# bowang-lab/BioReason

Measured on NVIDIA H100. Metric: GRPO tokens/sec (rollout+update), higher is better.
Workload: dtype bf16

## Files before the change

### bioreason_b200/csrc/br_common.cuh

```cuda
#pragma once
#include <cuda_runtime.h>
#include <cuda_bf16.h>
#include <cuda.h>
#include <stdint.h>
#include <stdio.h>
#include <string.h>
#include <stdlib.h>

#define BR_OK 0
#define BR_ERR_INVALID (-1)
#define BR_ERR_CUDA (-2)
#define BR_ERR_UNSUPPORTED (-3)

void br_set_error(const char* fmt, ...);

#define BR_CHECK_ARG(cond, ...)                     \
    do {                                            \
        if (!(cond)) {                              \
            br_set_error(__VA_ARGS__);              \
            return BR_ERR_INVALID;                  \
        }                                           \
    } while (0)

#define BR_CHECK_CUDA(expr)                                                              \
    do {                                                                                 \
        cudaError_t _e = (expr);                                                         \
        if (_e != cudaSuccess) {                                                         \
            br_set_error("%s failed: %s (%s:%d)", #expr, cudaGetErrorString(_e), __FILE__, __LINE__); \
            return BR_ERR_CUDA;                                                          \
        }                                                                                \
    } while (0)

#define BR_CHECK_LAUNCH() BR_CHECK_CUDA(cudaGetLastError())

static inline int br_num_sms() {
    static int n = 0;
    if (!n) {
        int dev = 0;
        cudaGetDevice(&dev);
        cudaDeviceGetAttribute(&n, cudaDevAttrMultiProcessorCount, dev);
        if (n <= 0) n = 132;
    }
    return n;
}

typedef __nv_bfloat16 bf16;
typedef __nv_bfloat162 bf162;

#ifdef __CUDACC__
namespace br {

__device__ __forceinline__ uint32_t smem_u32(const void* p) { return (uint32_t)__cvta_generic_to_shared(p); }
__device__ __forceinline__ int lane_id() { return threadIdx.x & 31; }

__device__ __forceinline__ void mbar_init(uint64_t* bar, uint32_t count) {
    asm volatile("mbarrier.init.shared::cta.b64 [%0], %1;" ::"r"(smem_u32(bar)), "r"(count));
}
__device__ __forceinline__ void mbar_fence_init() { asm volatile("fence.mbarrier_init.release.cluster;" ::: "memory"); }
__device__ __forceinline__ void mbar_expect_tx(uint64_t* bar, uint32_t bytes) {
    asm volatile("mbarrier.arrive.expect_tx.shared::cta.b64 _, [%0], %1;" ::"r"(smem_u32(bar)), "r"(bytes) : "memory");
}
__device__ __forceinline__ void mbar_arrive(uint64_t* bar) {
    asm volatile("mbarrier.arrive.shared::cta.b64 _, [%0];" ::"r"(smem_u32(bar)) : "memory");
}
__device__ __forceinline__ void mbar_wait(uint64_t* bar, uint32_t parity) {
    asm volatile(
        "{\n"
        ".reg .pred p;\n"
        "WAIT_%=:\n"
        "mbarrier.try_wait.parity.shared::cta.b64 p, [%0], %1;\n"
        "@p bra DONE_%=;\n"
        "bra WAIT_%=;\n"
        "DONE_%=:\n"
        "}\n" ::"r"(smem_u32(bar)),
        "r"(parity)
        : "memory");
}

__device__ __forceinline__ void tma_prefetch_desc(const void* tmap) {
    asm volatile("prefetch.tensormap [%0];" ::"l"(tmap) : "memory");
}
__device__ __forceinline__ void tma_load_2d(void* smem_dst, const void* tmap, uint64_t* bar, int c0, int c1) {
    asm volatile(
        "cp.async.bulk.tensor.2d.shared::cluster.global.mbarrier::complete_tx::bytes [%0], [%1, {%3, %4}], [%2];" ::"r"(
            smem_u32(smem_dst)),
        "l"(tmap), "r"(smem_u32(bar)), "r"(c0), "r"(c1)
        : "memory");
}

__device__ __forceinline__ void tma_load_2d_hint(void* smem_dst, const void* tmap, uint64_t* bar, int c0, int c1, uint64_t policy) {
    asm volatile(
        "cp.async.bulk.tensor.2d.shared::cluster.global.mbarrier::complete_tx::bytes.L2::cache_hint [%0], [%1, {%3, %4}], [%2], %5;" ::"r"(
            smem_u32(smem_dst)),
        "l"(tmap), "r"(smem_u32(bar)), "r"(c0), "r"(c1), "l"(policy)
        : "memory");
}
__device__ __forceinline__ void bulk_load_hint(void* smem_dst, const void* src, uint32_t bytes, uint64_t* bar, uint64_t policy) {
    asm volatile(
        "cp.async.bulk.shared::cluster.global.mbarrier::complete_tx::bytes.L2::cache_hint [%0], [%1], %2, [%3], %4;" ::"r"(smem_u32(smem_dst)),
        "l"(src), "r"(bytes), "r"(smem_u32(bar)), "l"(policy)
        : "memory");
}
__device__ __forceinline__ uint64_t make_policy_evict_first() {
    uint64_t p; asm volatile("createpolicy.fractional.L2::evict_first.b64 %0, 1.0;" : "=l"(p)); return p;
}

__device__ __forceinline__ void fence_proxy_async_smem() { asm volatile("fence.proxy.async.shared::cta;" ::: "memory"); }

__device__ __forceinline__ void launch_dependents() { asm volatile("griddepcontrol.launch_dependents;" ::: "memory"); }
__device__ __forceinline__ void grid_dep_wait() { asm volatile("griddepcontrol.wait;" ::: "memory"); }

__device__ __forceinline__ float warp_sum(float v) {
#pragma unroll
    for (int o = 16; o > 0; o >>= 1) v += __shfl_xor_sync(0xffffffffu, v, o);
    return v;
}
__device__ __forceinline__ float warp_max(float v) {
#pragma unroll
    for (int o = 16; o > 0; o >>= 1) v = fmaxf(v, __shfl_xor_sync(0xffffffffu, v, o));
    return v;
}
__device__ __forceinline__ uint32_t pack_bf16(float lo, float hi) {
    bf162 t = __floats2bfloat162_rn(lo, hi);
    return *reinterpret_cast<uint32_t*>(&t);
}
__device__ __forceinline__ float2 unpack_bf16(uint32_t v) {
    bf162 t = *reinterpret_cast<bf162*>(&v);
    return __bfloat1622float2(t);
}

__device__ __forceinline__ uint4 philox4x32_10(uint4 c, uint32_t k0, uint32_t k1) {
#pragma unroll
    for (int i = 0; i < 10; ++i) {
        if (i) { k0 += 0x9E3779B9u; k1 += 0xBB67AE85u; }
        const uint32_t hi0 = __umulhi(0xD2511F53u, c.x), lo0 = 0xD2511F53u * c.x;
        const uint32_t hi1 = __umulhi(0xCD9E8D57u, c.z), lo1 = 0xCD9E8D57u * c.z;
        c = make_uint4(hi1 ^ c.y ^ k0, lo1, hi0 ^ c.w ^ k1, lo0);
    }
    return c;
}

}
#endif

#ifdef __CUDACC__
template <typename... KArgs, typename... Args>
static inline cudaError_t br_launch_pdl(void (*kern)(KArgs...), dim3 grid, dim3 block, size_t smem, cudaStream_t st, Args&&... args) {
    cudaLaunchConfig_t cfg = {};
    cfg.gridDim = grid; cfg.blockDim = block; cfg.dynamicSmemBytes = smem; cfg.stream = st;
    static const bool no_pdl = getenv("BR_NO_PDL") != nullptr;
    cudaLaunchAttribute attr[1];
    attr[0].id = cudaLaunchAttributeProgrammaticStreamSerialization;
    attr[0].val.programmaticStreamSerializationAllowed = 1;
    cfg.attrs = attr; cfg.numAttrs = no_pdl ? 0 : 1;
    return cudaLaunchKernelEx(&cfg, kern, static_cast<KArgs>(args)...);
}
#endif

int br_make_tmap_2d_bf16(CUtensorMap* out, const void* base, uint64_t rows, uint64_t cols, uint64_t ld_elems, uint32_t box_rows);
```

### bioreason_b200/csrc/gemm_tc5.cu

```cuda
#include "br_common.cuh"
#include "../../include/bioreason_b200.h"
#include "lora_dropout.cuh"
#include "wgmma.cuh"

namespace {

constexpr int BM = 128;
constexpr int BK = 64;
constexpr int NTHREADS = 288;

enum { MODE_STD = 0, MODE_LSE = 1, MODE_DLOGITS = 2 };

struct GemmParams {
    int M, N, K, K2;
    int ldd;
    void* D;
    const void* bias; int bias_f32;
    const bf16* residual; long long ldr;
    float alpha;
    int act;
    int out_f32;
    const int* row_map;
    bf16* aux; long long ld_aux;
    const int* target;
    float* pmax; float* psum; float* tgt_logit;
    const float* lse; const float* gscale;
    int n_tiles_m, n_tiles_n;
    int group_m;
    br::DropParams drop;
};

template <int BN>
struct SmemLayout {
    static constexpr int A_BYTES = BM * BK * 2;
    static constexpr int B_BYTES = BN * BK * 2;
    static constexpr int STAGE_BYTES = A_BYTES + B_BYTES;
    static constexpr int NSTAGE = BN == 128 ? 6 : 4;
    static constexpr int TILE_BYTES = NSTAGE * STAGE_BYTES;
    static constexpr int TOTAL = TILE_BYTES + 256 + 1024;
};

__device__ __forceinline__ void tile_coords(int tile, int ntm, int ntn, int GROUP_M, int& mb, int& nb) {
    int per_group = GROUP_M * ntn;
    int g = tile / per_group;
    int first_m = g * GROUP_M;
    int gsize = min(GROUP_M, ntm - first_m);
    int r = tile - g * per_group;
    mb = first_m + (r % gsize);
    nb = r / gsize;
}

__device__ __forceinline__ float rbf(float x) { return __bfloat162float(__float2bfloat16(x)); }

template <int BN>
__device__ __forceinline__ void masked_segment(float (&acc)[BN / 2], uint64_t adesc, uint64_t bdesc, int k0, int mb, int nb, int wg,
                                               const GemmParams& p) {
    const int lane = threadIdx.x & 31, q = lane & 3;
    const long long grow = p.drop.row0 + mb * BM + wg * 64 + ((threadIdx.x >> 5) & 3) * 16 + (lane >> 2);
    const int cg0 = (nb * BN) >> 3;
    br::wg_wait<0>();
    br::wg_fence_operand(acc);
    for (int kk = 0; kk < BK / 16;) {
        const int kc = k0 + 16 * kk;
        if (kc >= p.K2) break;
        const int jb = kc / p.drop.r;
        const int nk = min(p.drop.r - (kc - jb * p.drop.r), BK - 16 * kk) >> 4;
        float tmp[BN / 2];
#pragma unroll
        for (int i = 0; i < BN / 2; ++i) tmp[i] = 0.f;
        br::wg_fence();
        for (int t = 0; t < nk; ++t) br::wgmma_ss<BN>(tmp, adesc + 2 * (kk + t), bdesc + 2 * (kk + t), 1);
        br::wg_commit();
        br::wg_wait<0>();
        br::wg_fence_operand(tmp);
        const int j = p.drop.proj + jb;
#pragma unroll
        for (int set = 0; set < BN / 16; ++set) {
            uint32_t w[4];
            br::quad_words(br::drop_group(p.drop, grow + 8 * (q & 1), cg0 + 2 * set + (q >> 1), j), w);
#pragma unroll
            for (int g = 0; g < 4; ++g) {
                const int e = 4 * (2 * set + (g >> 1)) + 2 * (g & 1);
                acc[e] += br::keep_lo(w[g], p.drop.T) ? tmp[e] * p.drop.inv_keep : 0.f;
                acc[e + 1] += br::keep_hi(w[g], p.drop.T) ? tmp[e + 1] * p.drop.inv_keep : 0.f;
            }
        }
        kk += nk;
    }
}

template <int BN, int MODE, bool MASK>
__global__ void __launch_bounds__(NTHREADS, 1)
gemm_tc5_kernel(const __grid_constant__ CUtensorMap tmA, const __grid_constant__ CUtensorMap tmB,
                const __grid_constant__ CUtensorMap tmA2, const __grid_constant__ CUtensorMap tmB2,
                const GemmParams p) {
    static_assert(BN == 128 || BN == 256, "tile width");
    static_assert(!MASK || BN == 128, "the masked LoRA segment runs on 128-wide tiles");
    constexpr int NSUB = BN / 128;
    using L = SmemLayout<BN>;
    extern __shared__ uint8_t smem_raw[];
    uint8_t* smem = reinterpret_cast<uint8_t*>((reinterpret_cast<uintptr_t>(smem_raw) + 1023) & ~uintptr_t(1023));
    uint64_t* full_bar = reinterpret_cast<uint64_t*>(smem + L::TILE_BYTES);
    uint64_t* empty_bar = full_bar + L::NSTAGE;

    const int warp = threadIdx.x >> 5;
    const int lane = threadIdx.x & 31;
    const int num_tiles = p.n_tiles_m * ((p.n_tiles_n + NSUB - 1) / NSUB);
    const int kb1 = (p.K + BK - 1) / BK;
    const int kb2 = (p.K2 + BK - 1) / BK;
    const int num_kb = kb1 + kb2;

    if (threadIdx.x == 0) {
        br::tma_prefetch_desc(&tmA);
        br::tma_prefetch_desc(&tmB);
        if (kb2) { br::tma_prefetch_desc(&tmA2); br::tma_prefetch_desc(&tmB2); }
        for (int s = 0; s < L::NSTAGE; ++s) { br::mbar_init(&full_bar[s], 1); br::mbar_init(&empty_bar[s], 2); }
        br::mbar_fence_init();
    }
    __syncthreads();

    if (warp == 8) {
        if (lane == 0) {
            int s = 0; uint32_t ph = 0;
            for (int tile = blockIdx.x; tile < num_tiles; tile += gridDim.x) {
                int mb, nb; tile_coords(tile, p.n_tiles_m, (p.n_tiles_n + NSUB - 1) / NSUB, p.group_m, mb, nb);
                for (int kb = 0; kb < num_kb; ++kb) {
                    br::mbar_wait(&empty_bar[s], ph ^ 1);
                    uint8_t* sa = smem + s * L::STAGE_BYTES;
                    uint8_t* sb = sa + L::A_BYTES;
                    br::mbar_expect_tx(&full_bar[s], L::STAGE_BYTES);
                    if (kb < kb1) {
                        br::tma_load_2d(sa, &tmA, &full_bar[s], kb * BK, mb * BM);
                        br::tma_load_2d(sb, &tmB, &full_bar[s], kb * BK, nb * BN);
                    } else {
                        br::tma_load_2d(sa, &tmA2, &full_bar[s], (kb - kb1) * BK, mb * BM);
                        br::tma_load_2d(sb, &tmB2, &full_bar[s], (kb - kb1) * BK, nb * BN);
                    }
                    if (++s == L::NSTAGE) { s = 0; ph ^= 1; }
                }
            }
        }
        return;
    }
    const int wg = warp >> 2;
    const int wt = threadIdx.x & 127;
    int s = 0; uint32_t ph = 0;
    for (int tile = blockIdx.x; tile < num_tiles; tile += gridDim.x) {
        int mb, nb; tile_coords(tile, p.n_tiles_m, (p.n_tiles_n + NSUB - 1) / NSUB, p.group_m, mb, nb);
        float acc[BN / 2];
#pragma unroll
        for (int i = 0; i < BN / 2; ++i) acc[i] = 0.f;
        int prev = 0;
        for (int kb = 0; kb < num_kb; ++kb) {
            br::mbar_wait(&full_bar[s], ph);
            const uint32_t sa = br::smem_u32(smem + s * L::STAGE_BYTES);
            const uint64_t adesc = br::wg_desc_k(sa + wg * 64 * 128);
            const uint64_t bdesc = br::wg_desc_k(sa + L::A_BYTES);
            if constexpr (MASK) {
                if (kb >= kb1) {
                    masked_segment<BN>(acc, adesc, bdesc, (kb - kb1) * BK, mb, nb, wg, p);
                    if (wt == 0) br::mbar_arrive(&empty_bar[prev]);
                    prev = s;
                    if (++s == L::NSTAGE) { s = 0; ph ^= 1; }
                    continue;
                }
            }
            br::wg_fence();
#pragma unroll
            for (int k = 0; k < BK / 16; ++k) br::wgmma_ss<BN>(acc, adesc + 2 * k, bdesc + 2 * k, 1);
            br::wg_commit();
            if (kb > 0) {
                br::wg_wait<1>();
                if (wt == 0) br::mbar_arrive(&empty_bar[prev]);
            }
            prev = s;
            if (++s == L::NSTAGE) { s = 0; ph ^= 1; }
        }
        br::wg_wait<0>();
        br::wg_fence_operand(acc);
        if (wt == 0) br::mbar_arrive(&empty_bar[prev]);

        const int r0 = mb * BM + wg * 64 + (warp & 3) * 16 + (lane >> 2);
        const int n0 = nb * BN;
        const int cq = 2 * (lane & 3);
        if constexpr (MODE == MODE_STD) {
#pragma unroll
            for (int hh = 0; hh < 2; ++hh) {
                const int row = r0 + 8 * hh;
                if (row >= p.M) continue;
                const long long orow = p.row_map ? (long long)p.row_map[row] : (long long)row;
                if (orow < 0) continue;
                float v[BN / 4];
#pragma unroll
                for (int i = 0; i < BN / 8; ++i) {
                    v[2 * i] = acc[4 * i + 2 * hh] * p.alpha;
                    v[2 * i + 1] = acc[4 * i + 2 * hh + 1] * p.alpha;
                    const int col = n0 + 8 * i + cq;
                    if (p.bias && n0 + 8 * i < p.N) {
                        if (p.bias_f32) {
                            const float* b = reinterpret_cast<const float*>(p.bias) + col;
                            v[2 * i] += __ldg(b); v[2 * i + 1] += __ldg(b + 1);
                        } else {
                            const bf16* b = reinterpret_cast<const bf16*>(p.bias) + col;
                            v[2 * i] += __bfloat162float(b[0]); v[2 * i + 1] += __bfloat162float(b[1]);
                        }
                    }
                }
                if (p.act == 1) {
#pragma unroll
                    for (int j = 0; j < BN / 16; ++j) {
                        if (n0 + 16 * j >= p.N) break;
                        if (p.aux) {
                            bf16* a = p.aux + orow * p.ld_aux + n0 + 16 * j + cq;
                            *reinterpret_cast<uint32_t*>(a) = br::pack_bf16(v[4 * j], v[4 * j + 1]);
                            *reinterpret_cast<uint32_t*>(a + 8) = br::pack_bf16(v[4 * j + 2], v[4 * j + 3]);
                        }
                        float o[2];
#pragma unroll
                        for (int e = 0; e < 2; ++e) {
                            const float g = rbf(v[4 * j + e]), u = rbf(v[4 * j + 2 + e]);
                            o[e] = rbf(g / (1.f + __expf(-g))) * u;
                        }
                        bf16* d = reinterpret_cast<bf16*>(p.D) + orow * (long long)p.ldd + (n0 >> 1) + 8 * j + cq;
                        *reinterpret_cast<uint32_t*>(d) = br::pack_bf16(o[0], o[1]);
                    }
                    continue;
                }
#pragma unroll
                for (int i = 0; i < BN / 8; ++i) {
                    if (n0 + 8 * i >= p.N) break;
                    const int col = n0 + 8 * i + cq;
                    float x0 = v[2 * i], x1 = v[2 * i + 1];
                    if (p.residual) {
                        const float2 r = br::unpack_bf16(__ldg(reinterpret_cast<const unsigned int*>(p.residual + orow * p.ldr + col)));
                        x0 = rbf(x0) + r.x; x1 = rbf(x1) + r.y;
                    }
                    if (p.out_f32) *reinterpret_cast<float2*>(reinterpret_cast<float*>(p.D) + orow * (long long)p.ldd + col) = make_float2(x0, x1);
                    else *reinterpret_cast<uint32_t*>(reinterpret_cast<bf16*>(p.D) + orow * (long long)p.ldd + col) = br::pack_bf16(x0, x1);
                }
            }
        } else if constexpr (MODE == MODE_LSE) {
#pragma unroll
            for (int h = 0; h < NSUB; ++h) {
                const int nh = n0 + 128 * h;
                if (NSUB > 1 && nh >= p.N) break;
#pragma unroll
                for (int hh = 0; hh < 2; ++hh) {
                    const int row = r0 + 8 * hh;
                    const bool row_ok = row < p.M;
                    const int tgt = row_ok ? p.target[row] : -1;
                    float mx = -INFINITY;
#pragma unroll
                    for (int i = 0; i < 16; ++i)
                        if (nh + 8 * i < p.N) mx = fmaxf(mx, fmaxf(acc[64 * h + 4 * i + 2 * hh], acc[64 * h + 4 * i + 2 * hh + 1]) * p.alpha);
                    mx = fmaxf(mx, __shfl_xor_sync(0xffffffffu, mx, 1));
                    mx = fmaxf(mx, __shfl_xor_sync(0xffffffffu, mx, 2));
                    float sm = 0.f;
#pragma unroll
                    for (int i = 0; i < 16; ++i) {
                        if (nh + 8 * i >= p.N) continue;
                        const int col = nh + 8 * i + cq;
                        const float x0 = acc[64 * h + 4 * i + 2 * hh] * p.alpha, x1 = acc[64 * h + 4 * i + 2 * hh + 1] * p.alpha;
                        sm += __expf(x0 - mx) + __expf(x1 - mx);
                        if (col == tgt) p.tgt_logit[row] = x0;
                        if (col + 1 == tgt) p.tgt_logit[row] = x1;
                    }
                    sm += __shfl_xor_sync(0xffffffffu, sm, 1);
                    sm += __shfl_xor_sync(0xffffffffu, sm, 2);
                    if (row_ok && (lane & 3) == 0) {
                        p.pmax[(long long)row * p.n_tiles_n + nb * NSUB + h] = mx;
                        p.psum[(long long)row * p.n_tiles_n + nb * NSUB + h] = sm;
                    }
                }
            }
        } else {
#pragma unroll
            for (int hh = 0; hh < 2; ++hh) {
                const int row = r0 + 8 * hh;
                if (row >= p.M) continue;
                const int tgt = p.target[row];
                const float lse = p.lse[row], gs = p.gscale[row];
#pragma unroll
                for (int i = 0; i < BN / 8; ++i) {
                    if (n0 + 8 * i >= p.N) break;
                    const int col = n0 + 8 * i + cq;
                    const float d0 = gs * ((col == tgt ? 1.f : 0.f) - __expf(acc[4 * i + 2 * hh] * p.alpha - lse));
                    const float d1 = gs * ((col + 1 == tgt ? 1.f : 0.f) - __expf(acc[4 * i + 2 * hh + 1] * p.alpha - lse));
                    *reinterpret_cast<uint32_t*>(reinterpret_cast<bf16*>(p.D) + (long long)row * p.ldd + col) = br::pack_bf16(d0, d1);
                }
            }
        }
    }
}

__global__ void lse_combine_kernel(const float* __restrict__ pmax, const float* __restrict__ psum, const float* __restrict__ tgt_logit,
                                   const int* __restrict__ target, int M, int nt, float* __restrict__ lse, float* __restrict__ logp) {
    int row = blockIdx.x * (blockDim.x >> 5) + (threadIdx.x >> 5);
    if (row >= M) return;
    int lane = threadIdx.x & 31;
    float mx = -INFINITY;
    for (int t = lane; t < nt; t += 32) mx = fmaxf(mx, pmax[(long long)row * nt + t]);
    mx = br::warp_max(mx);
    float s = 0.f;
    for (int t = lane; t < nt; t += 32) s += psum[(long long)row * nt + t] * __expf(pmax[(long long)row * nt + t] - mx);
    s = br::warp_sum(s);
    if (lane == 0) {
        float l = logf(s) + mx;
        if (lse) lse[row] = l;
        if (logp) logp[row] = (target[row] >= 0) ? tgt_logit[row] - l : 0.f;
    }
}

typedef CUresult (*PFN_encodeTiled)(CUtensorMap*, CUtensorMapDataType, cuuint32_t, void*, const cuuint64_t*, const cuuint64_t*,
                                    const cuuint32_t*, const cuuint32_t*, CUtensorMapInterleave, CUtensorMapSwizzle,
                                    CUtensorMapL2promotion, CUtensorMapFloatOOBfill);
PFN_encodeTiled get_encode() {
    static PFN_encodeTiled fn = nullptr;
    if (!fn) {
        void* f = nullptr;
        cudaDriverEntryPointQueryResult q;
        if (cudaGetDriverEntryPoint("cuTensorMapEncodeTiled", &f, cudaEnableDefault, &q) == cudaSuccess && q == cudaDriverEntryPointSuccess)
            fn = reinterpret_cast<PFN_encodeTiled>(f);
    }
    return fn;
}

template <int BN, int MODE, bool MASK = false>
int launch(const CUtensorMap& a, const CUtensorMap& b, const CUtensorMap& a2, const CUtensorMap& b2, const GemmParams& p, cudaStream_t st) {
    auto kern = gemm_tc5_kernel<BN, MODE, MASK>;
    static bool attr_set = false;
    if (!attr_set) {
        BR_CHECK_CUDA(cudaFuncSetAttribute(kern, cudaFuncAttributeMaxDynamicSharedMemorySize, SmemLayout<BN>::TOTAL));
        attr_set = true;
    }
    int tiles = p.n_tiles_m * ((p.n_tiles_n + BN / 128 - 1) / (BN / 128));
    int grid = tiles < br_num_sms() ? tiles : br_num_sms();
    kern<<<grid, NTHREADS, SmemLayout<BN>::TOTAL, st>>>(a, b, a2, b2, p);
    BR_CHECK_LAUNCH();
    return BR_OK;
}

template <int BN>
int launch_mode(int mode, const CUtensorMap& a, const CUtensorMap& b, const CUtensorMap& a2, const CUtensorMap& b2, const GemmParams& p,
                cudaStream_t st) {
    if (mode == MODE_STD) return launch<BN, MODE_STD>(a, b, a2, b2, p, st);
    if (mode == MODE_LSE) return launch<BN, MODE_LSE>(a, b, a2, b2, p, st);
    return launch<BN, MODE_DLOGITS>(a, b, a2, b2, p, st);
}

int run_gemm(int mode, const void* A, int64_t lda, const void* B, int64_t ldb, int M, int N, int K, const void* A2, int64_t lda2,
             const void* B2, int64_t ldb2, int K2, GemmParams& p, cudaStream_t st, bool masked = false) {
    BR_CHECK_ARG(M > 0 && N > 0 && K > 0, "gemm: empty problem M=%d N=%d K=%d", M, N, K);
    BR_CHECK_ARG(N % 8 == 0 && K % 8 == 0 && lda % 8 == 0 && ldb % 8 == 0, "gemm: N, K, lda, ldb must be multiples of 8");
    BR_CHECK_ARG(((uintptr_t)A % 16 == 0) && ((uintptr_t)B % 16 == 0), "gemm: operands must be 16-byte aligned");
    p.M = M; p.N = N; p.K = K; p.K2 = (A2 && B2) ? K2 : 0;
    p.n_tiles_m = (M + BM - 1) / BM;
    p.n_tiles_n = (N + 127) / 128;
    const bool wide = !masked && N >= 256 && K >= 512 && (long long)p.n_tiles_m * ((N + 255) / 256) >= 2ll * br_num_sms();
    const int bn = wide ? 256 : 128;
    {
        const long long a_block = (long long)BM * (K + p.K2) * 2;
        long long g = (16ll << 20) / (a_block > 0 ? a_block : 1);
        if (g < 8) g = 8;
        if (g > p.n_tiles_m) g = p.n_tiles_m;
        p.group_m = (int)g;
    }
    CUtensorMap ta, tb, ta2, tb2;
    int rc;
    if ((rc = br_make_tmap_2d_bf16(&ta, A, M, K, lda, BM))) return rc;
    if ((rc = br_make_tmap_2d_bf16(&tb, B, N, K, ldb, bn))) return rc;
    if (p.K2) {
        BR_CHECK_ARG(K2 % 8 == 0 && lda2 % 8 == 0 && ldb2 % 8 == 0, "gemm: K2, lda2, ldb2 must be multiples of 8");
        if ((rc = br_make_tmap_2d_bf16(&ta2, A2, M, K2, lda2, BM))) return rc;
        if ((rc = br_make_tmap_2d_bf16(&tb2, B2, N, K2, ldb2, bn))) return rc;
    } else { ta2 = ta; tb2 = tb; }
    if (masked) return launch<128, MODE_STD, true>(ta, tb, ta2, tb2, p, st);
    return wide ? launch_mode<256>(mode, ta, tb, ta2, tb2, p, st) : launch_mode<128>(mode, ta, tb, ta2, tb2, p, st);
}

}

int br_make_tmap_2d_bf16(CUtensorMap* out, const void* base, uint64_t rows, uint64_t cols, uint64_t ld_elems, uint32_t box_rows) {
    PFN_encodeTiled enc = get_encode();
    if (!enc) { br_set_error("cuTensorMapEncodeTiled not available from the driver"); return BR_ERR_CUDA; }
    cuuint64_t gdim[2] = {cols, rows};
    cuuint64_t gstr[1] = {ld_elems * 2};
    cuuint32_t box[2] = {64, box_rows};
    cuuint32_t estr[2] = {1, 1};
    CUresult r = enc(out, CU_TENSOR_MAP_DATA_TYPE_BFLOAT16, 2, const_cast<void*>(base), gdim, gstr, box, estr, CU_TENSOR_MAP_INTERLEAVE_NONE,
                     CU_TENSOR_MAP_SWIZZLE_128B, CU_TENSOR_MAP_L2_PROMOTION_L2_256B, CU_TENSOR_MAP_FLOAT_OOB_FILL_NONE);
    if (r != CUDA_SUCCESS) {
        br_set_error("cuTensorMapEncodeTiled failed (%d) rows=%llu cols=%llu ld=%llu box_rows=%u base=%p", (int)r, (unsigned long long)rows,
                     (unsigned long long)cols, (unsigned long long)ld_elems, box_rows, base);
        return BR_ERR_CUDA;
    }
    return BR_OK;
}

extern "C" {

int br_gemm_bf16(const void* A, int64_t lda, const void* B, int64_t ldb, void* D, int64_t ldd, int M, int N, int K,
                 const br_gemm_epilogue* e, void* stream) {
    GemmParams p;
    memset(&p, 0, sizeof(p));
    p.D = D; p.ldd = (int)ldd; p.alpha = 1.f;
    const void *A2 = nullptr, *B2 = nullptr; int64_t lda2 = 0, ldb2 = 0; int K2 = 0;
    bool masked = false;
    if (e) {
        p.bias = e->bias; p.bias_f32 = e->bias_dtype == BR_F32;
        p.residual = reinterpret_cast<const bf16*>(e->residual); p.ldr = e->ldr;
        p.alpha = e->alpha; p.act = e->act; p.out_f32 = e->out_dtype == BR_F32;
        p.row_map = e->row_map; p.aux = reinterpret_cast<bf16*>(e->aux_out); p.ld_aux = e->ld_aux;
        A2 = e->A2; B2 = e->B2; lda2 = e->lda2; ldb2 = e->ldb2; K2 = e->K2;
        BR_CHECK_ARG(!(p.act == 1 && (p.out_f32 || p.residual)), "gemm: gated-SiLU epilogue writes bf16 without residual");
        BR_CHECK_ARG(!(p.act == 1 && N % 16 != 0), "gemm: gated-SiLU epilogue needs N %% 16 == 0");
        if (e->lora_dropout) {
            int rc;
            if ((rc = br::check_drop(e->lora_dropout, "gemm"))) return rc;
            const int r = e->lora_dropout->r;
            BR_CHECK_ARG(A2 && B2 && r % 16 == 0 && r > 0 && K2 % r == 0 && e->lora_dropout->proj + K2 / r <= 8,
                         "gemm: masked LoRA segment needs A2/B2 with K2 = n_proj * r, r %% 16 == 0 (K2=%d r=%d)", K2, r);
            BR_CHECK_ARG(!p.row_map, "gemm: masked LoRA segment indexes mask rows by input row; no row_map");
            p.drop = br::drop_params(*e->lora_dropout);
            masked = true;
        }
    }
    BR_CHECK_ARG(ldd % 8 == 0 && (uintptr_t)D % 16 == 0, "gemm: D must be 16-byte aligned with ldd %% 8 == 0");
    return run_gemm(MODE_STD, A, lda, B, ldb, M, N, K, A2, lda2, B2, ldb2, K2, p, (cudaStream_t)stream, masked);
}

int64_t br_lmhead_workspace_bytes(int M, int V) {
    int nt = (V + 127) / 128;
    return (int64_t)M * nt * 2 * sizeof(float) + (int64_t)M * sizeof(float);
}

int br_lmhead_logprob_fwd(const void* H, int64_t ldh, const void* W, int64_t ldw, const int32_t* target, int M, int V, int K, float scale,
                          float* logp, float* lse, void* workspace, void* stream) {
    GemmParams p;
    memset(&p, 0, sizeof(p));
    int nt_max = (V + 127) / 128;
    p.alpha = scale; p.target = target;
    p.pmax = reinterpret_cast<float*>(workspace);
    p.psum = p.pmax + (int64_t)M * nt_max;
    p.tgt_logit = p.psum + (int64_t)M * nt_max;
    cudaStream_t st = (cudaStream_t)stream;
    BR_CHECK_CUDA(cudaMemsetAsync(p.tgt_logit, 0, (size_t)M * sizeof(float), st));
    int rc = run_gemm(MODE_LSE, H, ldh, W, ldw, M, V, K, nullptr, 0, nullptr, 0, 0, p, st);
    if (rc) return rc;
    const int wpb = 8;
    lse_combine_kernel<<<(M + wpb - 1) / wpb, wpb * 32, 0, st>>>(p.pmax, p.psum, p.tgt_logit, target, M, p.n_tiles_n, lse, logp);
    BR_CHECK_LAUNCH();
    return BR_OK;
}

int br_lmhead_dlogits(const void* H, int64_t ldh, const void* W, int64_t ldw, const int32_t* target, const float* lse, const float* gscale,
                      int M, int V, int K, float scale, void* dlogits, int64_t ldd, void* stream) {
    GemmParams p;
    memset(&p, 0, sizeof(p));
    p.alpha = scale; p.target = target; p.lse = lse; p.gscale = gscale; p.D = dlogits; p.ldd = (int)ldd;
    BR_CHECK_ARG(ldd % 8 == 0, "lmhead_dlogits: ldd %% 8");
    return run_gemm(MODE_DLOGITS, H, ldh, W, ldw, M, V, K, nullptr, 0, nullptr, 0, 0, p, (cudaStream_t)stream);
}

}
```

Measured before the change: 1224.

## Add 2-CTA cluster ping-pong WGMMA GEMM with multicast B and vectorized epilogue

Adds a new persistent GEMM kernel for wide standard-mode GEMMs with K up to 4096. It pairs CTAs in a cluster of two that share the B tile through TMA multicast, and runs two consumer warpgroups in ping-pong on alternating tiles so one tile's epilogue overlaps the other's MMA. Register reallocation via setmaxnreg favours the consumer warpgroups. The epilogue is factored out and now uses quad-shuffle transposes to emit 16-byte stores instead of 4-byte ones. This adds cross-CTA barrier complexity and lowers occupancy to one CTA per SM.

```diff
diff --git a/bioreason_b200/csrc/br_common.cuh b/bioreason_b200/csrc/br_common.cuh
--- a/bioreason_b200/csrc/br_common.cuh
+++ b/bioreason_b200/csrc/br_common.cuh
@@ -77,6 +77,20 @@
         : "memory");
 }
 
+__device__ __forceinline__ uint32_t cluster_ctarank() {
+    uint32_t r; asm volatile("mov.u32 %0, %%cluster_ctarank;" : "=r"(r)); return r;
+}
+__device__ __forceinline__ void cluster_sync() { asm volatile("barrier.cluster.arrive;\nbarrier.cluster.wait;" ::: "memory"); }
+__device__ __forceinline__ void mbar_arrive_cluster(uint64_t* bar, uint32_t cta) {
+    asm volatile("{\n.reg .b32 ra;\nmapa.shared::cluster.u32 ra, %0, %1;\nmbarrier.arrive.shared::cluster.b64 _, [ra];\n}" ::"r"(
+                     smem_u32(bar)), "r"(cta)
+                 : "memory");
+}
+template <int R> __device__ __forceinline__ void setmaxnreg_inc() { asm volatile("setmaxnreg.inc.sync.aligned.u32 %0;" ::"n"(R)); }
+template <int R> __device__ __forceinline__ void setmaxnreg_dec() { asm volatile("setmaxnreg.dec.sync.aligned.u32 %0;" ::"n"(R)); }
+__device__ __forceinline__ void named_sync(int id, int count) { asm volatile("bar.sync %0, %1;" ::"r"(id), "r"(count) : "memory"); }
+__device__ __forceinline__ void named_arrive(int id, int count) { asm volatile("bar.arrive %0, %1;" ::"r"(id), "r"(count) : "memory"); }
+
 __device__ __forceinline__ void tma_prefetch_desc(const void* tmap) {
     asm volatile("prefetch.tensormap [%0];" ::"l"(tmap) : "memory");
 }
@@ -99,6 +113,13 @@
     asm volatile(
         "cp.async.bulk.shared::cluster.global.mbarrier::complete_tx::bytes.L2::cache_hint [%0], [%1], %2, [%3], %4;" ::"r"(smem_u32(smem_dst)),
         "l"(src), "r"(bytes), "r"(smem_u32(bar)), "l"(policy)
+        : "memory");
+}
+__device__ __forceinline__ void tma_load_2d_mcast(void* smem_dst, const void* tmap, uint64_t* bar, int c0, int c1, uint16_t cta_mask) {
+    asm volatile(
+        "cp.async.bulk.tensor.2d.shared::cluster.global.mbarrier::complete_tx::bytes.multicast::cluster [%0], [%1, {%3, %4}], [%2], %5;" ::"r"(
+            smem_u32(smem_dst)),
+        "l"(tmap), "r"(smem_u32(bar)), "r"(c0), "r"(c1), "h"(cta_mask)
         : "memory");
 }
 __device__ __forceinline__ uint64_t make_policy_evict_first() {
diff --git a/bioreason_b200/csrc/gemm_tc5.cu b/bioreason_b200/csrc/gemm_tc5.cu
--- a/bioreason_b200/csrc/gemm_tc5.cu
+++ b/bioreason_b200/csrc/gemm_tc5.cu
@@ -40,6 +40,15 @@
     static constexpr int TOTAL = TILE_BYTES + 256 + 1024;
 };
 
+struct PpLayout {
+    static constexpr int A_BYTES = 64 * BK * 2;
+    static constexpr int B_BYTES = 256 * BK * 2;
+    static constexpr int STAGE_BYTES = A_BYTES + B_BYTES;
+    static constexpr int NSTAGE = 5;
+    static constexpr int TILE_BYTES = NSTAGE * STAGE_BYTES;
+    static constexpr int TOTAL = TILE_BYTES + 256 + 1024;
+};
+
 __device__ __forceinline__ void tile_coords(int tile, int ntm, int ntn, int GROUP_M, int& mb, int& nb) {
     int per_group = GROUP_M * ntn;
     int g = tile / per_group;
@@ -51,6 +60,19 @@
 }
 
 __device__ __forceinline__ float rbf(float x) { return __bfloat162float(__float2bfloat16(x)); }
+
+__device__ __forceinline__ void quad_transpose(float (&x)[4], int q) {
+#pragma unroll
+    for (int j = 0; j < 4; j += 2) {
+        const float r = __shfl_xor_sync(0xffffffffu, (q & 1) ? x[j] : x[j + 1], 1);
+        if (q & 1) x[j] = r; else x[j + 1] = r;
+    }
+#pragma unroll
+    for (int j = 0; j < 2; ++j) {
+        const float r = __shfl_xor_sync(0xffffffffu, (q & 2) ? x[j] : x[j + 2], 2);
+        if (q & 2) x[j] = r; else x[j + 2] = r;
+    }
+}
 
 template <int BN>
 __device__ __forceinline__ void masked_segment(float (&acc)[BN / 2], uint64_t adesc, uint64_t bdesc, int k0, int mb, int nb, int wg,
@@ -86,6 +108,154 @@
             }
         }
         kk += nk;
+    }
+}
+
+template <int BN, int MODE>
+__device__ __forceinline__ void epilogue(float (&acc)[BN / 2], const GemmParams& p, int r0, int nb) {
+    const int lane = threadIdx.x & 31;
+    const int q = lane & 3;
+    const int cq = 2 * q;
+    const int n0 = nb * BN;
+    constexpr int NSUB = BN / 128;
+    if constexpr (MODE == MODE_STD) {
+        auto value = [&](int i, int hh, float& v0, float& v1) {
+            v0 = acc[4 * i + 2 * hh] * p.alpha;
+            v1 = acc[4 * i + 2 * hh + 1] * p.alpha;
+            const int col = n0 + 8 * i + cq;
+            if (p.bias && n0 + 8 * i < p.N) {
+                if (p.bias_f32) {
+                    const float* b = reinterpret_cast<const float*>(p.bias) + col;
+                    v0 += __ldg(b); v1 += __ldg(b + 1);
+                } else {
+                    const bf16* b = reinterpret_cast<const bf16*>(p.bias) + col;
+                    v0 += __bfloat162float(b[0]); v1 += __bfloat162float(b[1]);
+                }
+            }
+        };
+#pragma unroll
+        for (int hh = 0; hh < 2; ++hh) {
+            const int row = r0 + 8 * hh;
+            const long long orow = row >= p.M ? -1ll : p.row_map ? (long long)p.row_map[row] : (long long)row;
+            if (p.act == 1) {
+#pragma unroll
+                for (int g4 = 0; g4 < BN / 64; ++g4) {
+                    float w[4];
+#pragma unroll
+                    for (int t = 0; t < 4; ++t) {
+                        const int j = 4 * g4 + t;
+                        float g[2], u[2], o[2];
+                        value(2 * j, hh, g[0], g[1]);
+                        value(2 * j + 1, hh, u[0], u[1]);
+                        if (p.aux && n0 + 16 * j < p.N) {
+                            bf16* a = p.aux + orow * p.ld_aux + n0 + 16 * j + cq;
+                            if (orow >= 0) {
+                                *reinterpret_cast<uint32_t*>(a) = br::pack_bf16(g[0], g[1]);
+                                *reinterpret_cast<uint32_t*>(a + 8) = br::pack_bf16(u[0], u[1]);
+                            }
+                        }
+#pragma unroll
+                        for (int e = 0; e < 2; ++e) {
+                            const float gb = rbf(g[e]), ub = rbf(u[e]);
+                            o[e] = rbf(gb / (1.f + __expf(-gb))) * ub;
+                        }
+                        w[t] = __uint_as_float(br::pack_bf16(o[0], o[1]));
+                    }
+                    quad_transpose(w, q);
+                    if (orow >= 0 && n0 + 16 * (4 * g4 + q) < p.N) {
+                        bf16* d = reinterpret_cast<bf16*>(p.D) + orow * (long long)p.ldd + (n0 >> 1) + 32 * g4 + 8 * q;
+                        *reinterpret_cast<uint4*>(d) = make_uint4(__float_as_uint(w[0]), __float_as_uint(w[1]), __float_as_uint(w[2]),
+                                                                  __float_as_uint(w[3]));
+                    }
+                }
+                continue;
+            }
+#pragma unroll
+            for (int g4 = 0; g4 < BN / 32; ++g4) {
+                float x[4], y[4];
+#pragma unroll
+                for (int t = 0; t < 4; ++t) value(4 * g4 + t, hh, x[t], y[t]);
+                quad_transpose(x, q);
+                quad_transpose(y, q);
+                const int col = n0 + 32 * g4 + 8 * q;
+                if (orow < 0 || col >= p.N) continue;
+                if (p.residual) {
+                    const unsigned int* rp = reinterpret_cast<const unsigned int*>(p.residual + orow * p.ldr + col);
+#pragma unroll
+                    for (int t = 0; t < 4; ++t) {
+                        const float2 r = br::unpack_bf16(__ldg(rp + t));
+                        x[t] = rbf(x[t]) + r.x; y[t] = rbf(y[t]) + r.y;
+                    }
+                }
+                if (p.out_f32) {
+                    float4* d = reinterpret_cast<float4*>(reinterpret_cast<float*>(p.D) + orow * (long long)p.ldd + col);
+                    d[0] = make_float4(x[0], y[0], x[1], y[1]);
+                    d[1] = make_float4(x[2], y[2], x[3], y[3]);
+                } else {
+                    *reinterpret_cast<uint4*>(reinterpret_cast<bf16*>(p.D) + orow * (long long)p.ldd + col) =
+                        make_uint4(br::pack_bf16(x[0], y[0]), br::pack_bf16(x[1], y[1]), br::pack_bf16(x[2], y[2]), br::pack_bf16(x[3], y[3]));
+                }
+            }
+        }
+    } else if constexpr (MODE == MODE_LSE) {
+#pragma unroll
+        for (int h = 0; h < NSUB; ++h) {
+            const int nh = n0 + 128 * h;
+            if (NSUB > 1 && nh >= p.N) break;
+#pragma unroll
+            for (int hh = 0; hh < 2; ++hh) {
+                const int row = r0 + 8 * hh;
+                const bool row_ok = row < p.M;
+                const int tgt = row_ok ? p.target[row] : -1;
+                float mx = -INFINITY;
+#pragma unroll
+                for (int i = 0; i < 16; ++i)
+                    if (nh + 8 * i < p.N) mx = fmaxf(mx, fmaxf(acc[64 * h + 4 * i + 2 * hh], acc[64 * h + 4 * i + 2 * hh + 1]) * p.alpha);
+                mx = fmaxf(mx, __shfl_xor_sync(0xffffffffu, mx, 1));
+                mx = fmaxf(mx, __shfl_xor_sync(0xffffffffu, mx, 2));
+                float sm = 0.f;
+#pragma unroll
+                for (int i = 0; i < 16; ++i) {
+                    if (nh + 8 * i >= p.N) continue;
+                    const int col = nh + 8 * i + cq;
+                    const float x0 = acc[64 * h + 4 * i + 2 * hh] * p.alpha, x1 = acc[64 * h + 4 * i + 2 * hh + 1] * p.alpha;
+                    sm += __expf(x0 - mx) + __expf(x1 - mx);
+                    if (col == tgt) p.tgt_logit[row] = x0;
+                    if (col + 1 == tgt) p.tgt_logit[row] = x1;
+                }
+                sm += __shfl_xor_sync(0xffffffffu, sm, 1);
+                sm += __shfl_xor_sync(0xffffffffu, sm, 2);
+                if (row_ok && (lane & 3) == 0) {
+                    p.pmax[(long long)row * p.n_tiles_n + nb * NSUB + h] = mx;
+                    p.psum[(long long)row * p.n_tiles_n + nb * NSUB + h] = sm;
+                }
+            }
+        }
+    } else {
+#pragma unroll
+        for (int hh = 0; hh < 2; ++hh) {
+            const int row = r0 + 8 * hh;
+            const bool row_ok = row < p.M;
+            const int tgt = row_ok ? p.target[row] : -1;
+            const float lse = row_ok ? p.lse[row] : 0.f, gs = row_ok ? p.gscale[row] : 0.f;
+#pragma unroll
+            for (int g4 = 0; g4 < BN / 32; ++g4) {
+                float w[4];
+#pragma unroll
+                for (int t = 0; t < 4; ++t) {
+                    const int i = 4 * g4 + t;
+                    const int col = n0 + 8 * i + cq;
+                    const float d0 = gs * ((col == tgt ? 1.f : 0.f) - __expf(acc[4 * i + 2 * hh] * p.alpha - lse));
+                    const float d1 = gs * ((col + 1 == tgt ? 1.f : 0.f) - __expf(acc[4 * i + 2 * hh + 1] * p.alpha - lse));
+                    w[t] = __uint_as_float(br::pack_bf16(d0, d1));
+                }
+                quad_transpose(w, q);
+                const int col = n0 + 32 * g4 + 8 * q;
+                if (row_ok && col < p.N)
+                    *reinterpret_cast<uint4*>(reinterpret_cast<bf16*>(p.D) + (long long)row * p.ldd + col) =
+                        make_uint4(__float_as_uint(w[0]), __float_as_uint(w[1]), __float_as_uint(w[2]), __float_as_uint(w[3]));
+            }
+        }
     }
 }
 
@@ -179,118 +349,106 @@
         br::wg_wait<0>();
         br::wg_fence_operand(acc);
         if (wt == 0) br::mbar_arrive(&empty_bar[prev]);
-
-        const int r0 = mb * BM + wg * 64 + (warp & 3) * 16 + (lane >> 2);
-        const int n0 = nb * BN;
-        const int cq = 2 * (lane & 3);
-        if constexpr (MODE == MODE_STD) {
-#pragma unroll
-            for (int hh = 0; hh < 2; ++hh) {
-                const int row = r0 + 8 * hh;
-                if (row >= p.M) continue;
-                const long long orow = p.row_map ? (long long)p.row_map[row] : (long long)row;
-                if (orow < 0) continue;
-                float v[BN / 4];
-#pragma unroll
-                for (int i = 0; i < BN / 8; ++i) {
-                    v[2 * i] = acc[4 * i + 2 * hh] * p.alpha;
-                    v[2 * i + 1] = acc[4 * i + 2 * hh + 1] * p.alpha;
-                    const int col = n0 + 8 * i + cq;
-                    if (p.bias && n0 + 8 * i < p.N) {
-                        if (p.bias_f32) {
-                            const float* b = reinterpret_cast<const float*>(p.bias) + col;
-                            v[2 * i] += __ldg(b); v[2 * i + 1] += __ldg(b + 1);
-                        } else {
-                            const bf16* b = reinterpret_cast<const bf16*>(p.bias) + col;
-                            v[2 * i] += __bfloat162float(b[0]); v[2 * i + 1] += __bfloat162float(b[1]);
-                        }
+        epilogue<BN, MODE>(acc, p, mb * BM + wg * 64 + (warp & 3) * 16 + (lane >> 2), nb);
+    }
+}
+
+constexpr int PP_THREADS = 384;
+constexpr int PP_ORDER_BAR = 1;
+
+__global__ void __launch_bounds__(PP_THREADS, 1)
+gemm_pp_kernel(const __grid_constant__ CUtensorMap tmA, const __grid_constant__ CUtensorMap tmB,
+               const __grid_constant__ CUtensorMap tmA2, const __grid_constant__ CUtensorMap tmB2,
+               const GemmParams p) {
+    constexpr int BN = 256;
+    using L = PpLayout;
+    extern __shared__ uint8_t smem_raw[];
+    uint8_t* smem = reinterpret_cast<uint8_t*>((reinterpret_cast<uintptr_t>(smem_raw) + 1023) & ~uintptr_t(1023));
+    uint64_t* full_bar = reinterpret_cast<uint64_t*>(smem + L::TILE_BYTES);
+    uint64_t* empty_bar = full_bar + L::NSTAGE;
+
+    const uint32_t rank = br::cluster_ctarank();
+    const int cluster = blockIdx.x >> 1, n_clusters = gridDim.x >> 1;
+    const int ntn = (p.n_tiles_n + 1) / 2;
+    const int num_tiles = p.n_tiles_m * ntn;
+    const int kb1 = (p.K + BK - 1) / BK;
+    const int kb2 = (p.K2 + BK - 1) / BK;
+    const int num_kb = kb1 + kb2;
+
+    if (threadIdx.x == 0) {
+        br::tma_prefetch_desc(&tmA);
+        br::tma_prefetch_desc(&tmB);
+        if (kb2) { br::tma_prefetch_desc(&tmA2); br::tma_prefetch_desc(&tmB2); }
+        for (int s = 0; s < L::NSTAGE; ++s) { br::mbar_init(&full_bar[s], 1); br::mbar_init(&empty_bar[s], 2); }
+        br::mbar_fence_init();
+    }
+    br::cluster_sync();
+
+    const int wgi = threadIdx.x >> 7;
+    if (wgi == 0) {
+        br::setmaxnreg_dec<40>();
+        if (threadIdx.x == 0) {
+            int s = 0; uint32_t ph = 0;
+            for (int tile = cluster; tile < num_tiles; tile += n_clusters) {
+                int mb, nb; tile_coords(tile, p.n_tiles_m, ntn, p.group_m, mb, nb);
+                const int arow = min(mb * BM + 64 * (int)rank, p.M - 1);
+                const int brow = min(nb * BN + 128 * (int)rank, p.N - 1);
+                for (int kb = 0; kb < num_kb; ++kb) {
+                    br::mbar_wait(&empty_bar[s], ph ^ 1);
+                    uint8_t* sa = smem + s * L::STAGE_BYTES;
+                    uint8_t* sb = sa + L::A_BYTES + rank * (L::B_BYTES / 2);
+                    br::mbar_expect_tx(&full_bar[s], L::STAGE_BYTES);
+                    if (kb < kb1) {
+                        br::tma_load_2d(sa, &tmA, &full_bar[s], kb * BK, arow);
+                        br::tma_load_2d_mcast(sb, &tmB, &full_bar[s], kb * BK, brow, 0x3);
+                    } else {
+                        br::tma_load_2d(sa, &tmA2, &full_bar[s], (kb - kb1) * BK, arow);
+                        br::tma_load_2d_mcast(sb, &tmB2, &full_bar[s], (kb - kb1) * BK, brow, 0x3);
                     }
-                }
-                if (p.act == 1) {
-#pragma unroll
-                    for (int j = 0; j < BN / 16; ++j) {
-                        if (n0 + 16 * j >= p.N) break;
-                        if (p.aux) {
-                            bf16* a = p.aux + orow * p.ld_aux + n0 + 16 * j + cq;
-                            *reinterpret_cast<uint32_t*>(a) = br::pack_bf16(v[4 * j], v[4 * j + 1]);
-                            *reinterpret_cast<uint32_t*>(a + 8) = br::pack_bf16(v[4 * j + 2], v[4 * j + 3]);
-                        }
-                        float o[2];
-#pragma unroll
-                        for (int e = 0; e < 2; ++e) {
-                            const float g = rbf(v[4 * j + e]), u = rbf(v[4 * j + 2 + e]);
-                            o[e] = rbf(g / (1.f + __expf(-g))) * u;
-                        }
-                        bf16* d = reinterpret_cast<bf16*>(p.D) + orow * (long long)p.ldd + (n0 >> 1) + 8 * j + cq;
-                        *reinterpret_cast<uint32_t*>(d) = br::pack_bf16(o[0], o[1]);
-                    }
-                    continue;
-                }
-#pragma unroll
-                for (int i = 0; i < BN / 8; ++i) {
-                    if (n0 + 8 * i >= p.N) break;
-                    const int col = n0 + 8 * i + cq;
-                    float x0 = v[2 * i], x1 = v[2 * i + 1];
-                    if (p.residual) {
-                        const float2 r = br::unpack_bf16(__ldg(reinterpret_cast<const unsigned int*>(p.residual + orow * p.ldr + col)));
-                        x0 = rbf(x0) + r.x; x1 = rbf(x1) + r.y;
-                    }
-                    if (p.out_f32) *reinterpret_cast<float2*>(reinterpret_cast<float*>(p.D) + orow * (long long)p.ldd + col) = make_float2(x0, x1);
-                    else *reinterpret_cast<uint32_t*>(reinterpret_cast<bf16*>(p.D) + orow * (long long)p.ldd + col) = br::pack_bf16(x0, x1);
-                }
-            }
-        } else if constexpr (MODE == MODE_LSE) {
-#pragma unroll
-            for (int h = 0; h < NSUB; ++h) {
-                const int nh = n0 + 128 * h;
-                if (NSUB > 1 && nh >= p.N) break;
-#pragma unroll
-                for (int hh = 0; hh < 2; ++hh) {
-                    const int row = r0 + 8 * hh;
-                    const bool row_ok = row < p.M;
-                    const int tgt = row_ok ? p.target[row] : -1;
-                    float mx = -INFINITY;
-#pragma unroll
-                    for (int i = 0; i < 16; ++i)
-                        if (nh + 8 * i < p.N) mx = fmaxf(mx, fmaxf(acc[64 * h + 4 * i + 2 * hh], acc[64 * h + 4 * i + 2 * hh + 1]) * p.alpha);
-                    mx = fmaxf(mx, __shfl_xor_sync(0xffffffffu, mx, 1));
-                    mx = fmaxf(mx, __shfl_xor_sync(0xffffffffu, mx, 2));
-                    float sm = 0.f;
-#pragma unroll
-                    for (int i = 0; i < 16; ++i) {
-                        if (nh + 8 * i >= p.N) continue;
-                        const int col = nh + 8 * i + cq;
-                        const float x0 = acc[64 * h + 4 * i + 2 * hh] * p.alpha, x1 = acc[64 * h + 4 * i + 2 * hh + 1] * p.alpha;
-                        sm += __expf(x0 - mx) + __expf(x1 - mx);
-                        if (col == tgt) p.tgt_logit[row] = x0;
-                        if (col + 1 == tgt) p.tgt_logit[row] = x1;
-                    }
-                    sm += __shfl_xor_sync(0xffffffffu, sm, 1);
-                    sm += __shfl_xor_sync(0xffffffffu, sm, 2);
-                    if (row_ok && (lane & 3) == 0) {
-                        p.pmax[(long long)row * p.n_tiles_n + nb * NSUB + h] = mx;
-                        p.psum[(long long)row * p.n_tiles_n + nb * NSUB + h] = sm;
-                    }
-                }
-            }
-        } else {
-#pragma unroll
-            for (int hh = 0; hh < 2; ++hh) {
-                const int row = r0 + 8 * hh;
-                if (row >= p.M) continue;
-                const int tgt = p.target[row];
-                const float lse = p.lse[row], gs = p.gscale[row];
-#pragma unroll
-                for (int i = 0; i < BN / 8; ++i) {
-                    if (n0 + 8 * i >= p.N) break;
-                    const int col = n0 + 8 * i + cq;
-                    const float d0 = gs * ((col == tgt ? 1.f : 0.f) - __expf(acc[4 * i + 2 * hh] * p.alpha - lse));
-                    const float d1 = gs * ((col + 1 == tgt ? 1.f : 0.f) - __expf(acc[4 * i + 2 * hh + 1] * p.alpha - lse));
-                    *reinterpret_cast<uint32_t*>(reinterpret_cast<bf16*>(p.D) + (long long)row * p.ldd + col) = br::pack_bf16(d0, d1);
-                }
-            }
-        }
-    }
+                    if (++s == L::NSTAGE) { s = 0; ph ^= 1; }
+                }
+            }
+        }
+    } else {
+        br::setmaxnreg_inc<232>();
+        const int c = wgi - 1;
+        const int warp = (threadIdx.x >> 5) & 3;
+        const int lane = threadIdx.x & 31;
+        const int wt = threadIdx.x & 127;
+        const uint32_t peer = rank ^ 1;
+        int j = c;
+        for (int tile = cluster + c * n_clusters; tile < num_tiles; tile += 2 * n_clusters, j += 2) {
+            int mb, nb; tile_coords(tile, p.n_tiles_m, ntn, p.group_m, mb, nb);
+            float acc[BN / 2];
+#pragma unroll
+            for (int i = 0; i < BN / 2; ++i) acc[i] = 0.f;
+            if (j > 0) br::named_sync(PP_ORDER_BAR + c, 256);
+            int pos = j * num_kb;
+            int prev = 0;
+            for (int kb = 0; kb < num_kb; ++kb, ++pos) {
+                const int s = pos % L::NSTAGE;
+                br::mbar_wait(&full_bar[s], (pos / L::NSTAGE) & 1);
+                const uint32_t sa = br::smem_u32(smem + s * L::STAGE_BYTES);
+                const uint64_t adesc = br::wg_desc_k(sa);
+                const uint64_t bdesc = br::wg_desc_k(sa + L::A_BYTES);
+                br::wg_fence();
+#pragma unroll
+                for (int k = 0; k < BK / 16; ++k) br::wgmma_ss<BN>(acc, adesc + 2 * k, bdesc + 2 * k, 1);
+                br::wg_commit();
+                if (kb > 0) {
+                    br::wg_wait<1>();
+                    if (wt == 0) { br::mbar_arrive(&empty_bar[prev]); br::mbar_arrive_cluster(&empty_bar[prev], peer); }
+                }
+                prev = s;
+            }
+            if (tile + n_clusters < num_tiles) br::named_arrive(PP_ORDER_BAR + (c ^ 1), 256);
+            br::wg_wait<0>();
+            br::wg_fence_operand(acc);
+            if (wt == 0) { br::mbar_arrive(&empty_bar[prev]); br::mbar_arrive_cluster(&empty_bar[prev], peer); }
+            epilogue<BN, MODE_STD>(acc, p, mb * BM + 64 * (int)rank + warp * 16 + (lane >> 2), nb);
+        }
+    }
+    br::cluster_sync();
 }
 
 __global__ void lse_combine_kernel(const float* __restrict__ pmax, const float* __restrict__ psum, const float* __restrict__ tgt_logit,
@@ -340,6 +498,29 @@
     return BR_OK;
 }
 
+int launch_pp(const CUtensorMap& a, const CUtensorMap& b, const CUtensorMap& a2, const CUtensorMap& b2, const GemmParams& p, cudaStream_t st) {
+    auto kern = gemm_pp_kernel;
+    cudaLaunchConfig_t cfg = {};
+    cudaLaunchAttribute attr[1];
+    attr[0].id = cudaLaunchAttributeClusterDimension;
+    attr[0].val.clusterDim.x = 2; attr[0].val.clusterDim.y = 1; attr[0].val.clusterDim.z = 1;
+    cfg.blockDim = dim3(PP_THREADS);
+    cfg.dynamicSmemBytes = PpLayout::TOTAL;
+    cfg.stream = st;
+    cfg.attrs = attr; cfg.numAttrs = 1;
+    static int max_clusters = 0;
+    if (!max_clusters) {
+        BR_CHECK_CUDA(cudaFuncSetAttribute(kern, cudaFuncAttributeMaxDynamicSharedMemorySize, PpLayout::TOTAL));
+        cfg.gridDim = dim3(2 * (br_num_sms() / 2));
+        BR_CHECK_CUDA(cudaOccupancyMaxActiveClusters(&max_clusters, kern, &cfg));
+        BR_CHECK_ARG(max_clusters > 0, "gemm: no 2-CTA cluster of the 128 x 256 kernel fits on this device");
+    }
+    const int tiles = p.n_tiles_m * ((p.n_tiles_n + 1) / 2);
+    cfg.gridDim = dim3(2 * (tiles < max_clusters ? tiles : max_clusters));
+    BR_CHECK_CUDA(cudaLaunchKernelEx(&cfg, kern, a, b, a2, b2, p));
+    return BR_OK;
+}
+
 template <int BN>
 int launch_mode(int mode, const CUtensorMap& a, const CUtensorMap& b, const CUtensorMap& a2, const CUtensorMap& b2, const GemmParams& p,
                 cudaStream_t st) {
@@ -357,7 +538,9 @@
     p.n_tiles_m = (M + BM - 1) / BM;
     p.n_tiles_n = (N + 127) / 128;
     const bool wide = !masked && N >= 256 && K >= 512 && (long long)p.n_tiles_m * ((N + 255) / 256) >= 2ll * br_num_sms();
-    const int bn = wide ? 256 : 128;
+    const bool pingpong = wide && mode == MODE_STD && K + p.K2 <= 4096;
+    const int a_rows = pingpong ? 64 : BM;
+    const int b_rows = pingpong ? 128 : wide ? 256 : 128;
     {
         const long long a_block = (long long)BM * (K + p.K2) * 2;
         long long g = (16ll << 20) / (a_block > 0 ? a_block : 1);
@@ -367,14 +550,15 @@
     }
     CUtensorMap ta, tb, ta2, tb2;
     int rc;
-    if ((rc = br_make_tmap_2d_bf16(&ta, A, M, K, lda, BM))) return rc;
-    if ((rc = br_make_tmap_2d_bf16(&tb, B, N, K, ldb, bn))) return rc;
+    if ((rc = br_make_tmap_2d_bf16(&ta, A, M, K, lda, a_rows))) return rc;
+    if ((rc = br_make_tmap_2d_bf16(&tb, B, N, K, ldb, b_rows))) return rc;
     if (p.K2) {
         BR_CHECK_ARG(K2 % 8 == 0 && lda2 % 8 == 0 && ldb2 % 8 == 0, "gemm: K2, lda2, ldb2 must be multiples of 8");
-        if ((rc = br_make_tmap_2d_bf16(&ta2, A2, M, K2, lda2, BM))) return rc;
-        if ((rc = br_make_tmap_2d_bf16(&tb2, B2, N, K2, ldb2, bn))) return rc;
+        if ((rc = br_make_tmap_2d_bf16(&ta2, A2, M, K2, lda2, a_rows))) return rc;
+        if ((rc = br_make_tmap_2d_bf16(&tb2, B2, N, K2, ldb2, b_rows))) return rc;
     } else { ta2 = ta; tb2 = tb; }
     if (masked) return launch<128, MODE_STD, true>(ta, tb, ta2, tb2, p, st);
+    if (pingpong) return launch_pp(ta, tb, ta2, tb2, p, st);
     return wide ? launch_mode<256>(mode, ta, tb, ta2, tb2, p, st) : launch_mode<128>(mode, ta, tb, ta2, tb2, p, st);
 }
 
@@ -414,6 +598,7 @@
         A2 = e->A2; B2 = e->B2; lda2 = e->lda2; ldb2 = e->ldb2; K2 = e->K2;
         BR_CHECK_ARG(!(p.act == 1 && (p.out_f32 || p.residual)), "gemm: gated-SiLU epilogue writes bf16 without residual");
         BR_CHECK_ARG(!(p.act == 1 && N % 16 != 0), "gemm: gated-SiLU epilogue needs N %% 16 == 0");
+        BR_CHECK_ARG(!p.aux || ((uintptr_t)p.aux % 16 == 0 && p.ld_aux % 8 == 0), "gemm: aux_out must be 16-byte aligned with ld_aux %% 8 == 0");
         if (e->lora_dropout) {
             int rc;
             if ((rc = br::check_drop(e->lora_dropout, "gemm"))) return rc;
```

Measured after the change: 1224 (median of 6 runs). No clear change (+0.0%).
